# JuliaDSP/DSP.jl

Hardware: NVIDIA H100
Metric: Gsamples/s filt+welch on 2^26 cplx-F32 (higher is better)
Workload: dtype c64 (ComplexF32; f32 arithmetic)

## Files before the change

dsp.jl_b200/csrc/fft_core.cuh:

```cuda
#pragma once
#include "common.cuh"
#include <math.h>

#ifndef DSP_PROBE
#define DSP_PROBE 0
#endif

namespace dspb200 {

template <typename T> struct fft_pad { static constexpr int K = sizeof(T) == 4 ? 2 : 1; };
template <typename T> __host__ __device__ constexpr int fft_pad256(int n) {
    if (sizeof(T) == 4) return n == 512 ? 8 : (n == 1024 ? 4 : (n == 8192 ? 4 : 2));
    return n == 512 ? 4 : (n == 1024 ? 2 : (n == 8192 ? 2 : 1));
}
template <typename T> __host__ __device__ constexpr int fft_pad4096(int n) {
    if (sizeof(T) == 4) return n == 8192 ? 2 : (n == 16384 ? 4 : 0);
    return n == 8192 ? 1 : 0;
}
template <typename T, int N> __host__ __device__ __forceinline__ constexpr int padaddr(int p) {
    return p + fft_pad<T>::K * (p >> 4) + fft_pad256<T>(N) * (p >> 8) + fft_pad4096<T>(N) * (p >> 12);
}
template <typename T> __host__ __device__ constexpr int padded_len(int n) {
    return ((n - 1) + fft_pad<T>::K * ((n - 1) >> 4) + fft_pad256<T>(n) * ((n - 1) >> 8) + fft_pad4096<T>(n) * ((n - 1) >> 12) + 1 + 3) & ~3;
}
// ... 217 lines not shown
    if constexpr (fft_uses_t256<N>()) {
        for (int i = tid; i < fft_tw256_len(N); i += NT) s256[i] = g256[i];
    }
    if constexpr (fft_tl_in_smem<T, N>()) {
        cx<T>* sl = s256 + (fft_uses_t256<N>() ? fft_tw256_len(N) : 0);
        for (int i = tid; i < fft_tl_len<N>(); i += NT) sl[i] = gtl[i];
        c.tl = sl;
    }
    return c;
}
template <typename T, int N, int NT>
__device__ __forceinline__ FftCtx<T> fft_make_ctx(cx<T>* smem, const cx<T>* __restrict__ g16, const cx<T>* __restrict__ g256,
                                                    const cx<T>* __restrict__ gtl, int tid) {
    return fft_make_ctx_at<T, N, NT>(smem, smem + padded_len<T>(N), g16, g256, gtl, tid);
}

template <int NT> __device__ __forceinline__ void fft_group256_sync(int tid) {
#ifdef __CUDA_ARCH__
    if constexpr (NT <= 256) __syncthreads();
    else asm volatile("bar.sync %0, %1;" ::"r"(1 + (tid >> 8)), "r"(256) : "memory");
#endif
}

struct FftCtaScope {
    __device__ __forceinline__ void sync() const {
#ifdef __CUDA_ARCH__
        __syncthreads();
#endif
    }
};
template <int NTG> struct FftGroupScope {
    int id;
    __device__ __forceinline__ void sync() const {
#ifdef __CUDA_ARCH__
        asm volatile("bar.sync %0, %1;" ::"r"(id), "n"(NTG) : "memory");
#endif
    }
};

template <int NT> __device__ __forceinline__ void fft_gate_wait(int tid) {
#ifdef __CUDA_ARCH__
    if constexpr (NT > 256) {
        const int k = tid >> 8;
        if (k > 0) asm volatile("bar.sync %0, 512;" ::"r"(4 + k) : "memory");
    }
#endif
}
template <int NT> __device__ __forceinline__ void fft_gate_open(int tid) {
#ifdef __CUDA_ARCH__
    if constexpr (NT > 256) {
        const int k = tid >> 8;
        if (k < NT / 256 - 1) asm volatile("bar.arrive %0, 512;" ::"r"(5 + k) : "memory");
    }
#endif
}

template <typename T, int N> __host__ __device__ __forceinline__ void fft_store_block(cx<T>* sm, int cidx, const cx<T> (&v)[16]) {
    cx<T>* p = sm + padaddr<T, N>(16 * fft_block_of<N>(cidx));
#pragma unroll
    for (int r = 0; r < 16; r += 2) sts2<T>(p + r, v[r], v[r + 1]);
}

template <typename T, int N, int NT, bool SYNC, class Ld0, class Scope = FftCtaScope>
__host__ __device__ __forceinline__ void fft_first_pass(const FftCtx<T>& c, int tid, Ld0 ld0, Scope sc = Scope()) {
    constexpr int Q = fft_plan_traits<N>::Q;
    constexpr int ITERS = (Q + NT - 1) / NT;
#pragma unroll
    for (int it = 0; it < ITERS; ++it) {
        const int b = tid + it * NT;
        const bool active = (Q % NT == 0) || b < Q;
        cx<T> v[16];
        if (active) {
#pragma unroll
            for (int r = 0; r < 16; ++r) v[r] = ld0(b + r * Q, it, r);
            fft_bfly16_plain<T>(v);
        }
#ifdef __CUDA_ARCH__
        if constexpr (SYNC) { if (it == 0) sc.sync(); }
#endif
        if (active) fft_store_block<T, N>(c.sm, b, v);
    }
}

template <typename T, int N, int NT, bool SYNC, int ITERS, class Scope = FftCtaScope>
__device__ __forceinline__ void fft_first_pass_regs(const FftCtx<T>& c, int tid, cx<T> (&v)[ITERS][16], Scope sc = Scope()) {
    constexpr int Q = fft_plan_traits<N>::Q;
    static_assert(ITERS == (Q + NT - 1) / NT, "register tile does not match the thread count");
#pragma unroll
    for (int it = 0; it < ITERS; ++it) {
        const int b = tid + it * NT;
        const bool active = (Q % NT == 0) || b < Q;
        if (active) fft_bfly16_plain<T>(v[it]);
        if constexpr (SYNC) { if (it == 0) sc.sync(); }
        if (active) fft_store_block<T, N>(c.sm, b, v[it]);
    }
}

template <typename T, int N, int NT, int S, bool GATE = false>
__host__ __device__ __forceinline__ void fft_pass16(const FftCtx<T>& c, int tid) {
    static_assert(S == 16 || S == 256, "radix-16 pass with an unsupported stride");
    constexpr int Q = fft_plan_traits<N>::Q;
    constexpr int ITERS = (Q + NT - 1) / NT;
    constexpr int PS = padded_stride<T, N>(S);
    const cx<T>* tab = S == 16 ? c.t16 : c.t256;
    if constexpr (ITERS == 2 && Q % NT == 0) {
        const int b0 = tid, b1 = tid + NT;
        const int t0 = b0 & (S - 1), t1 = b1 & (S - 1);
        cx<T>* p0 = c.sm + padaddr<T, N>((b0 / S) * (16 * S) + t0);
        cx<T>* p1 = c.sm + padaddr<T, N>((b1 / S) * (16 * S) + t1);
        cx<T> v0[16], v1[16], w0[8], w1[8];
        if constexpr (GATE) fft_gate_wait<NT>(tid);
        load_tw8<T, S, fft_tw_row(N)>(tab, t0, w0);
#pragma unroll
        for (int r = 0; r < 16; ++r) v0[r] = p0[r * PS];
        load_tw8<T, S, fft_tw_row(N)>(tab, t1, w1);
#pragma unroll
        for (int r = 0; r < 16; ++r) v1[r] = p1[r * PS];
        if constexpr (GATE) fft_gate_open<NT>(tid);
        fft_bfly<T, 16, false>(v0, w0);
#pragma unroll
        for (int r = 0; r < 16; ++r) p0[r * PS] = v0[r];
        fft_bfly<T, 16, false>(v1, w1);
#pragma unroll
        for (int r = 0; r < 16; ++r) p1[r * PS] = v1[r];
        return;
    }
#pragma unroll 1
    for (int it = 0; it < ITERS; ++it) {
        const int b = tid + it * NT;
        if (Q % NT != 0 && b >= Q) break;
        const int t = b & (S - 1);
        cx<T>* p = c.sm + padaddr<T, N>((b / S) * (16 * S) + t);
        cx<T> v[16], w[8];
        if constexpr (GATE && ITERS == 1) fft_gate_wait<NT>(tid);
        load_tw8<T, S, fft_tw_row(N)>(tab, t, w);
#pragma unroll
        for (int r = 0; r < 16; ++r) v[r] = p[r * PS];
        if constexpr (GATE && ITERS == 1) fft_gate_open<NT>(tid);
        fft_bfly<T, 16, false>(v, w);
#pragma unroll
        for (int r = 0; r < 16; ++r) p[r * PS] = v[r];
    }
}

template <typename T, int N, int NT, class Scope = FftCtaScope>
__device__ __forceinline__ void fft_middle(const FftCtx<T>& c, int tid, Scope sc = Scope()) {
    constexpr int NMID = fft_plan_traits<N>::NMID;
    static_assert(NMID < 2 || std::is_same<Scope, FftCtaScope>::value, "thread groups run transforms of at most 4096 points");
    if constexpr (NMID >= 1) {
#if !(DSP_PROBE & 16)
        fft_pass16<T, N, NT, 16, true>(c, tid);
#endif
        if constexpr (NMID == 2) {
            fft_group256_sync<NT>(tid);
#if !(DSP_PROBE & 1)
            fft_pass16<T, N, NT, 256>(c, tid);
#endif
        }
        sc.sync();
    }
}

template <typename T, int N>
__host__ __device__ __forceinline__ void fft_last_pass_load(const FftCtx<T>& c, int tp, cx<T> (&v)[16]) {
    constexpr int Q = fft_plan_traits<N>::Q;
    const cx<T>* p = c.sm + padaddr<T, N>(tp);
#pragma unroll
    for (int r = 0; r < 16; ++r) v[r] = p[padaddr<T, N>(r * Q)];
}
template <typename T, int N>
__host__ __device__ __forceinline__ void fft_last_pass_bfly(const FftCtx<T>& c, int tp, cx<T> (&v)[16]) {
    using P = fft_plan_traits<N>;
    constexpr int Q = P::Q, RL = P::RL;
    if constexpr (RL == 16) {
        cx<T> w[8];
        load_tw8<T, Q, fft_tw_row(N)>(Q == 16 ? c.t16 : c.t256, tp, w);
        fft_bfly<T, 16, false>(v, w);
    } else {
        constexpr int NBF = 16 / RL;
        constexpr int TLK = P::TLK;
#pragma unroll
        for (int a = 0; a < NBF; ++a) {
            const int t = tp + Q * a;
            cx<T> w[RL / 2];
            if constexpr (N == 16384) {
                const cx<T> w1 = fft_tl_in_smem<T, N>() ? c.tl[t] : ldtw<T>(c.tl, t);
                w[1] = w1;
                w[0] = mkc<T>(fma_(w1.x, w1.x, -(w1.y * w1.y)), (w1.x + w1.x) * w1.y);
            } else {
#pragma unroll
                for (int i = 0; i < TLK; ++i) w[i] = fft_tl_in_smem<T, N>() ? c.tl[t * TLK + i] : ldtw<T>(c.tl, t * TLK + i);
            }
            cx<T> u[RL];
#pragma unroll
            for (int j = 0; j < RL; ++j) u[j] = v[a + NBF * j];
            fft_bfly<T, RL, false>(u, w);
#pragma unroll
            for (int j = 0; j < RL; ++j) v[a + NBF * j] = u[j];
        }
    }
}
template <typename T, int N, int GATE_NT = 0>
__host__ __device__ __forceinline__ void fft_last_pass(const FftCtx<T>& c, int tp, cx<T> (&v)[16], int tid = 0) {
    if constexpr (GATE_NT > 256) fft_gate_wait<GATE_NT>(tid);
    fft_last_pass_load<T, N>(c, tp, v);
    if constexpr (GATE_NT > 256) fft_gate_open<GATE_NT>(tid);
    fft_last_pass_bfly<T, N>(c, tp, v);
}

template <int N> struct fft_last_chunks {
    static constexpr int RL = fft_plan_traits<N>::RL;
    static constexpr int COUNT = 16 / RL;
};
template <typename T, int N, int A>
__device__ __forceinline__ void fft_last_pass_chunk(const FftCtx<T>& c, int tp, cx<T> (&u)[fft_plan_traits<N>::RL]) {
    using P = fft_plan_traits<N>;
    constexpr int Q = P::Q, RL = P::RL, NBF = 16 / RL;
    const cx<T>* p = c.sm + padaddr<T, N>(tp);
#pragma unroll
    for (int j = 0; j < RL; ++j) u[j] = p[padaddr<T, N>((A + NBF * j) * Q)];
    if constexpr (RL == 16) {
        cx<T> w[8];
        load_tw8<T, Q, fft_tw_row(N)>(Q == 16 ? c.t16 : c.t256, tp, w);
        fft_bfly<T, 16, false>(u, w);
    } else {
        const int t = tp + Q * A;
        cx<T> w[RL / 2];
        if constexpr (N == 16384) {
            const cx<T> w1 = fft_tl_in_smem<T, N>() ? c.tl[t] : ldtw<T>(c.tl, t);
            w[1] = w1;
            w[0] = mkc<T>(fma_(w1.x, w1.x, -(w1.y * w1.y)), (w1.x + w1.x) * w1.y);
        } else {
#pragma unroll
            for (int i = 0; i < P::TLK; ++i) w[i] = fft_tl_in_smem<T, N>() ? c.tl[t * P::TLK + i] : ldtw<T>(c.tl, t * P::TLK + i);
        }
        fft_bfly<T, RL, false>(u, w);
    }
}

template <typename T, int N, int NT, class Ld0, class StLast>
__device__ __forceinline__ void fft_forward(const FftCtx<T>& c, int tid, Ld0 ld0, StLast stlast) {
    constexpr int Q = fft_plan_traits<N>::Q;
    constexpr int ITERS = (Q + NT - 1) / NT;
    fft_first_pass<T, N, NT, false>(c, tid, ld0);
    __syncthreads();
    fft_middle<T, N, NT>(c, tid);
#pragma unroll
    for (int it = 0; it < ITERS; ++it) {
        const int tp = tid + it * NT;
        if (Q % NT != 0 && tp >= Q) break;
        cx<T> v[16];
        fft_last_pass<T, N>(c, tp, v);
#pragma unroll
        for (int r = 0; r < 16; ++r) stlast(tp + r * Q, it, r, v[r]);
    }
}

struct fft_r32 {
    static constexpr int N = 16384;
    static constexpr int NT = 512;
    static constexpr int Q = N / 32;
    static constexpr int QL = N / 16;
    static constexpr int T32_LEN = 32 * 16;
    static constexpr int TL_LEN = 2 * QL;
    static constexpr int TABLE_LEN = T32_LEN + TL_LEN;
    static constexpr int C10 = 2;
    static constexpr int PADDED_LEN = ((N - 1) + C10 * ((N - 1) >> 10) + 1 + 3) & ~3;
    static constexpr int SMEM_ELEMS = PADDED_LEN + TABLE_LEN;
};
__host__ __device__ __forceinline__ constexpr int fft_r32_padaddr(int p) { return p + fft_r32::C10 * (p >> 10); }
__host__ __device__ __forceinline__ constexpr int fft_r32_block_of(int c) { return 32 * (c & 15) + (c >> 4); }

template <typename T> struct FftR32Ctx {
    cx<T>* sm;
    const cx<T>* t32;
    const cx<T>* tl;
};
template <typename T>
__device__ __forceinline__ FftR32Ctx<T> fft_r32_make_ctx(cx<T>* data, cx<T>* tabs, const cx<T>* __restrict__ g, int tid) {
    for (int i = tid; i < fft_r32::TABLE_LEN; i += fft_r32::NT) tabs[i] = g[i];
    return FftR32Ctx<T>{data, tabs, tabs + fft_r32::T32_LEN};
}

// ... 125 lines not shown
```

dsp.jl_b200/csrc/spectral.cu:

```cuda
#include "fft_core.cuh"
#include "async_copy.cuh"
#include "cufft_exec.cuh"
#include <math.h>
#include <stdlib.h>
#include <new>
#include <vector>

namespace dspb200 {

struct SpecPlanImpl {
    int dtype = 0;
    bool cplx = false, f64 = false;
    int64_t n = 0, noverlap = 0, hop = 0, nfft = 0;
    int onesided = 0;
    int64_t nout = 0;
    bool fused = false;
    int device = 0;
    int sm_count = 0;
    void* d_window = nullptr;
    void* d_tw = nullptr;
    void* d_t32 = nullptr;
    void* d_t16 = nullptr;
    void* d_t256 = nullptr;
    size_t smem_optin = 0;
    int64_t ntapers = 0;
    DevBuf tmp;
    struct WelchCfg { void* kern = nullptr; size_t smem = 0; int g = 0, per_sm = 0, threads = 0, mode = -1; int64_t vctas = 0, used = 0; };
    WelchCfg welch_cfg[2];
    int nparts = 0;
    int rows_used = 0;
    DevBuf partial;
    WelchCfg welch_batch_cfg[2];
    WelchCfg welch_mt_cfg[2];
    DevBuf bpartial;
    DevBuf bacc;
    cufftHandle fft = 0;
    bool fft_ok = false;
    int64_t batch = 0;
    int64_t nbins_fft = 0;
    DevBuf segbuf, specbuf, acc;
    HostPipe pipe;
    DevBuf hin, hout;
    DevBuf seam;
    DevBuf y;
};

template <typename T> struct win_t { using type = double; };
template <> struct win_t<float> { using type = float2; };
__device__ __forceinline__ double win_mul(double v, double w) { return v * w; }
__device__ __forceinline__ float win_mul(float v, float2 w) { return fmaf(v, w.x, v * w.y); }

__device__ __forceinline__ float add_rn(float a, float b) { return __fadd_rn(a, b); }
__device__ __forceinline__ double add_rn(double a, double b) { return __dadd_rn(a, b); }

template <typename T, bool CPLX> struct in_type { using type = T; };
template <typename T> struct in_type<T, true> { using type = cx<T>; };

template <typename T, int N, bool CPLX, int MODE> struct welch_layout {
    using In = typename in_type<T, CPLX>::type;
    using W = typename win_t<T>::type;
    __host__ __device__ static size_t table_bytes() { return (size_t)fft_table_elems<T, N>() * sizeof(cx<T>); }
    __host__ __device__ static size_t window_bytes(int64_t n) { return MODE == 2 ? (size_t)n * sizeof(W) : 0; }
    __host__ __device__ static size_t stage_elems(int64_t n, int64_t hop) { return MODE >= 1 ? (size_t)(CPLX ? n : hop + n) : 0; }
    __host__ __device__ static size_t group_bytes(int64_t n, int64_t hop) {
        return (((size_t)padded_len<T>(N) * sizeof(cx<T>) + stage_elems(n, hop) * sizeof(In) + 15) & ~(size_t)15) + 16;
    }
    __host__ __device__ static size_t total(int64_t n, int64_t hop, int groups) {
        return table_bytes() + window_bytes(n) + (size_t)groups * group_bytes(n, hop);
    }
};
template <typename T, int N, int G> struct welch_bounds {
    static constexpr int NTG = fft_threads<N>::value;
    static constexpr int minblocks = G == 1 ? fft_minblocks<T, N>::value : 1;
};

struct Nil {};
template <bool USED, typename X> using welch_arg = typename std::conditional<USED, X, Nil>::type;

template <typename T, int N, bool CPLX, int MODE, int G, bool BATCH, bool TAPERS = false>
__global__ void __launch_bounds__((welch_bounds<T, N, G>::NTG * G), (welch_bounds<T, N, G>::minblocks))
welch_fused_kernel(const void* __restrict__ s_, welch_arg<BATCH, int64_t> chan_stride, welch_arg<!BATCH, int64_t> seg0,
                   int64_t nseg, welch_arg<BATCH, int64_t> upc, welch_arg<BATCH, int64_t> per, welch_arg<BATCH, int> slices,
                   welch_arg<BATCH, int64_t> nitems, int64_t hop, int n, welch_arg<!BATCH, int64_t> sample_offset,
                   const typename win_t<T>::type* __restrict__ win, const cx<T>* __restrict__ tw,
                   const cx<T>* __restrict__ g16, const cx<T>* __restrict__ g256, T* __restrict__ partial,
                   welch_arg<!BATCH, int> fresh_from) {
    constexpr int NT = fft_threads<N>::value;
    constexpr int NB16 = N / 16;
    constexpr int ITL = (NB16 + NT - 1) / NT;
    using L = welch_layout<T, N, CPLX, MODE>;
    using Scope = typename std::conditional<G == 1, FftCtaScope, FftGroupScope<NT>>::type;
    extern __shared__ __align__(16) unsigned char smem_raw[];
    using In = typename in_type<T, CPLX>::type;
    const In* s = reinterpret_cast<const In*>(s_);
    const int gid = G == 1 ? 0 : threadIdx.x / NT;
    const int tid = G == 1 ? threadIdx.x : threadIdx.x - gid * NT;
    constexpr bool TMA = MODE >= 1;
    constexpr bool WSM = MODE == 2;
    constexpr bool WREG = MODE == 3;
    static_assert(!TAPERS || (BATCH && MODE <= 1), "taper rows: the batched work assignment, window read per unit");
    using W = typename win_t<T>::type;
    cx<T>* tabs = reinterpret_cast<cx<T>*>(smem_raw);
    W* wsm = reinterpret_cast<W*>(smem_raw + L::table_bytes());
    unsigned char* gbase = smem_raw + L::table_bytes() + L::window_bytes(n) + (size_t)gid * L::group_bytes(n, hop);
    cx<T>* sm = reinterpret_cast<cx<T>*>(gbase);
    In* stage = reinterpret_cast<In*>(sm + padded_len<T>(N));
    uint64_t* bar = reinterpret_cast<uint64_t*>(gbase + L::group_bytes(n, hop) - 16);
    pdl_launch_dependents();
    const FftCtx<T> ctx = fft_make_ctx_at<T, N, NT * G>(sm, tabs, g16, g256, tw, threadIdx.x);
    if constexpr (WSM) {
        for (int i = threadIdx.x; i < n; i += NT * G) wsm[i] = win[i];
    }
    Scope scope;
    if constexpr (G > 1) scope.id = 8 + gid;
    W wreg[WREG ? ITL : 1][WREG ? 16 : 1];
    if constexpr (WREG) {
#pragma unroll
        for (int it = 0; it < ITL; ++it)
#pragma unroll
            for (int r = 0; r < 16; ++r) {
                const int j = tid + it * NT + r * NB16;
                wreg[it][r] = (j < n && tid + it * NT < NB16) ? win[j] : W{};
            }
    }

    T acc[ITL][16];
#pragma unroll
    for (int i = 0; i < ITL; ++i)
#pragma unroll
        for (int r = 0; r < 16; ++r) acc[i][r] = T(0);

    int64_t work;
    if constexpr (BATCH) work = nitems;
    else work = CPLX ? nseg : (nseg + 1) / 2;
    const int64_t vcta = (int64_t)blockIdx.x * G + gid, nvcta = (int64_t)gridDim.x * G;
    const int64_t share = (work + nvcta - 1) / nvcta;
    const int64_t w0 = vcta * share < work ? vcta * share : work;
    const int64_t w1 = w0 + share < work ? w0 + share : work;

    auto unit_src = [&](int64_t c, int64_t u) -> const In* {
        if constexpr (TAPERS) return s + c * chan_stride;
        else if constexpr (BATCH) return s + c * chan_stride + (CPLX ? u : 2 * u) * hop;
        else return s + ((seg0 + (CPLX ? u : 2 * u)) * hop - sample_offset);
    };
    auto unit_bytes = [&](int64_t u) -> uint32_t {
        const bool hasB = !CPLX && (2 * u + 1 < nseg);
        return (uint32_t)((hasB ? hop + n : n) * sizeof(In));
    };
    auto item_range = [&](int64_t i, int64_t& c, int64_t& ua, int64_t& ub) {
        if constexpr (BATCH) {
            c = i / slices;
            ua = (i - c * slices) * per;
            ub = ua + per < upc ? ua + per : upc;
        }
    };
    if constexpr (TMA) {
        if (tid == 0) {
            mbar_init(bar, 1);
            mbar_fence_init();
        }
    }
    pdl_wait();
    __syncthreads();
    int64_t c = 0, ua = BATCH ? 0 : w0, ub = BATCH ? 0 : w1;
    if constexpr (BATCH) {
        if (w0 < w1) item_range(w0, c, ua, ub);
    }
    if constexpr (TMA) {
        if (tid == 0 && w0 < w1) {
            mbar_expect_tx(bar, unit_bytes(ua));
            tma_load_1d(stage, unit_src(c, ua), unit_bytes(ua), bar);
        }
    }
    uint32_t parity = 0;

    for (int64_t item = w0; !BATCH || item < w1; ++item) {
        for (int64_t u = ua; u < ub; ++u) {
            const bool hasB = !CPLX && (2 * u + 1 < nseg);
            const In* pa = TMA ? stage : unit_src(c, u);
            const In* pb = pa + hop;
            const W* wu = TAPERS ? win + u * n : win;
            if constexpr (TMA) {
                if (!TAPERS || u == ua) {
                    mbar_wait(bar, parity);
                    parity ^= 1;
                }
            }
            auto ld0 = [&](int j, int it, int r) -> cx<T> {
                if (j >= n) return mkc<T>(T(0), T(0));
                if constexpr (CPLX) {
                    cx<T> v = pa[j];
                    if (WREG || WSM || wu) { const W w = WREG ? wreg[WREG ? it : 0][WREG ? r : 0] : (WSM ? wsm[j] : wu[j]); v = mkc<T>(win_mul(v.x, w), win_mul(v.y, w)); }
                    return v;
                } else {
                    T a = pa[j];
                    T b = hasB ? pb[j] : T(0);
                    if (WREG || WSM || wu) { const W w = WREG ? wreg[WREG ? it : 0][WREG ? r : 0] : (WSM ? wsm[j] : wu[j]); a = win_mul(a, w); b = win_mul(b, w); }
                    return mkc<T>(a, b);
                }
            };
            fft_first_pass<T, N, NT, true>(ctx, tid, ld0, scope);
            scope.sync();
            if constexpr (TMA && !BATCH) {
                if (tid == 0 && u + 1 < ub) {
                    fence_proxy_async_shared();
                    mbar_expect_tx(bar, unit_bytes(u + 1));
                    tma_load_1d(stage, unit_src(c, u + 1), unit_bytes(u + 1), bar);
                }
            }
            if constexpr (TMA && BATCH) {
                if (tid == 0) {
                    int64_t nc = c, nu = u + 1, nub = ub;
                    if (nu == ub && item + 1 < w1) item_range(item + 1, nc, nu, nub);
                    else if (TAPERS) nu = nub;
                    if (nu < nub) {
                        fence_proxy_async_shared();
                        mbar_expect_tx(bar, unit_bytes(nu));
                        tma_load_1d(stage, unit_src(nc, nu), unit_bytes(nu), bar);
                    }
                }
            }
            fft_middle<T, N, NT>(ctx, tid, scope);
#pragma unroll
            for (int it = 0; it < ITL; ++it) {
                const int tp = tid + it * NT;
                if (NB16 % NT != 0 && tp >= NB16) break;
                cx<T> v[16];
                fft_last_pass<T, N>(ctx, tp, v);
#pragma unroll
                for (int r = 0; r < 16; ++r) acc[it][r] += cabs2(v[r]);
            }
        }

        T* dst = partial + (BATCH ? item : vcta) * N;
        bool add = false;
        if constexpr (!BATCH) add = vcta < fresh_from;
#pragma unroll
        for (int it = 0; it < ITL; ++it) {
            const int tp = tid + it * NT;
            if (tp < NB16) {
#pragma unroll
                for (int r = 0; r < 16; ++r) {
                    if constexpr (BATCH) {
                        dst[tp + r * NB16] = acc[it][r];
                        acc[it][r] = T(0);
                    } else {
                        T* q = dst + tp + r * NB16;
                        *q = add ? *q + acc[it][r] : acc[it][r];
                    }
                }
            }
        }
        if constexpr (BATCH) {
            if (item + 1 < w1) item_range(item + 1, c, ua, ub);
        } else {
            break;
        }
    }
}

template <typename T, int N>
__global__ void __launch_bounds__(1024) welch_finalize_kernel(const T* __restrict__ partial, int rows, T* __restrict__ out,
                                                              int nout, int real_in, int onesided, double m1, double m2) {
    __shared__ double red[32][33];
    pdl_launch_dependents();
    pdl_wait();
    const int b = threadIdx.x & 31, sl = threadIdx.x >> 5, nw = blockDim.x >> 5;
    const int k = blockIdx.x * 32 + b;
    const T* chan = partial + (int64_t)blockIdx.y * rows * N;
    double sum = 0.0;
    if (k < nout) {
        const T* c0 = chan + k;
        const T* c1 = chan + ((N - k) & (N - 1));
        if (real_in) {
            for (int c = sl; c < rows; c += nw) sum += (double)c0[(int64_t)c * N] + (double)c1[(int64_t)c * N];
        } else {
            for (int c = sl; c < rows; c += nw) sum += (double)c0[(int64_t)c * N];
        }
    }
    red[sl][b] = sum;
    __syncthreads();
    if (sl == 0 && k < nout) {
        for (int i = 1; i < nw; ++i) sum += red[i][b];
        double m = m1;
        if (real_in) {
            sum *= 0.5;
// ... 631 lines not shown
        }
        red[which][sl][b] = sum;
    };
    part(rows, ri, 0);
    part(seam_rows, rs, 1);
    __syncthreads();
    if (sl == 0 && k < nout) {
        const int nwi = ri < 32 ? ri : 32, nws = rs < 32 ? rs : 32;
        double sum = red[0][0][b];
        for (int i = 1; i < nwi; ++i) sum += red[0][i][b];
        if (rs > 0) {
            double s2 = red[1][0][b];
            for (int i = 1; i < nws; ++i) s2 += red[1][i][b];
            sum += s2;
        }
        double* q = acc + (int64_t)blockIdx.y * nout + k;
        *q = add ? *q + sum : sum;
    }
}

template <typename T>
__global__ void welch_stream_acc_kernel(const cx<T>* __restrict__ X, int64_t nbins_fft, int64_t nfft, int64_t nout, int64_t f0,
                                        int64_t nf, int64_t k, int add, double* __restrict__ acc) {
    const int64_t kk = (int64_t)blockIdx.x * blockDim.x + threadIdx.x;
    if (kk >= nout) return;
    const int64_t c = f0 / k + blockIdx.y;
    const int64_t a = c * k > f0 ? c * k : f0, e = (c + 1) * k < f0 + nf ? (c + 1) * k : f0 + nf;
    const int64_t src = kk < nbins_fft ? kk : nfft - kk;
    double sum = 0.0;
    for (int64_t f = a; f < e; ++f) sum += (double)cabs2(X[(f - f0) * nbins_fft + src]);
    double* q = acc + c * nout + kk;
    *q = (add || a > c * k) ? *q + sum : sum;
}

template <typename T>
__global__ void welch_stream_power_kernel(const double* __restrict__ acc, int64_t nout, int64_t nfft, int onesided, int half,
                                          double m1, double m2, T* __restrict__ out) {
    const int64_t kk = (int64_t)blockIdx.x * blockDim.x + threadIdx.x;
    if (kk >= nout) return;
    const int64_t i = (int64_t)blockIdx.y * nout + kk;
    double sum = acc[i];
    if (half) sum *= 0.5;
    const double m = (onesided && kk != 0 && 2 * kk != nfft) ? m2 : m1;
    out[i] = (T)(sum * m);
}

static bool fused_size_ok(int64_t nfft, bool f64) {
    if (nfft < 256 || (nfft & (nfft - 1))) return false;
    return nfft <= (f64 ? 8192 : 16384);
}

template <typename T, typename F> static int fused_size_dispatch(const SpecPlanImpl* p, const char* what, F&& f) {
    switch (p->nfft) {
#define X(NN)                                                                                               \
    case NN:                                                                                                \
        if constexpr (sizeof(T) == 8 && NN > 8192) break;                                                   \
        else return f(T(0), std::integral_constant<int, NN>());
        X(256) X(512) X(1024) X(2048) X(4096) X(8192) X(16384)
#undef X
    }
    set_error("no fused %s kernel for nfft=%lld", what, (long long)p->nfft);
    return DSPB200_EUNSUPPORTED;
}
template <typename F> static int fused_dispatch(const SpecPlanImpl* p, const char* what, F&& f) {
    return p->f64 ? fused_size_dispatch<double>(p, what, f) : fused_size_dispatch<float>(p, what, f);
}

template <typename K> static int set_smem(K kernel, size_t bytes) {
    if (bytes > 48 * 1024) DSP_CUDA(cudaFuncSetAttribute(kernel, cudaFuncAttributeMaxDynamicSharedMemorySize, (int)bytes));
    return DSPB200_OK;
}

template <typename T, bool BATCH>
using welch_kern_t = void (*)(const void*, welch_arg<BATCH, int64_t>, welch_arg<!BATCH, int64_t>, int64_t,
                              welch_arg<BATCH, int64_t>, welch_arg<BATCH, int64_t>, welch_arg<BATCH, int>,
                              welch_arg<BATCH, int64_t>, int64_t, int, welch_arg<!BATCH, int64_t>,
                              const typename win_t<T>::type*, const cx<T>*, const cx<T>*, const cx<T>*, T*,
                              welch_arg<!BATCH, int>);

template <typename T, int N, bool CPLX, bool BATCH, bool TAPERS, typename F>
static int welch_candidates(const SpecPlanImpl* p, bool aligned, bool windowed, F&& f) {
    constexpr bool MULTI = sizeof(T) == 4 && N >= 1024 && N <= 4096;
    constexpr bool WREGOK = sizeof(T) == 4 && N <= 4096;
#define DSP_WELCH_CAND(MODE_, G_)                                                                                   \
    DSP_TRY(f(welch_kern_t<T, BATCH>(welch_fused_kernel<T, N, CPLX, MODE_, G_, BATCH, TAPERS>),                     \
              welch_layout<T, N, CPLX, MODE_>::total(p->n, p->hop, G_), MODE_, G_))
    if (aligned) {
        if constexpr (!TAPERS) {
            if (windowed) {
                if constexpr (CPLX) {
                    if constexpr (WREGOK) DSP_WELCH_CAND(3, 1);
                    DSP_WELCH_CAND(2, 1);
                    if constexpr (MULTI) { DSP_WELCH_CAND(3, 2); DSP_WELCH_CAND(2, 2); }
                } else {
                    if constexpr (MULTI) { DSP_WELCH_CAND(2, 3); DSP_WELCH_CAND(2, 2); }
                    DSP_WELCH_CAND(2, 1);
                    if constexpr (WREGOK) DSP_WELCH_CAND(3, 1);
                }
            }
        }
        if constexpr (MULTI && !CPLX) DSP_WELCH_CAND(1, 3);
        DSP_WELCH_CAND(1, 1);
        if constexpr (MULTI) DSP_WELCH_CAND(1, 2);
    }
    DSP_WELCH_CAND(0, 1);
#undef DSP_WELCH_CAND
    return DSPB200_OK;
}

template <typename K>
static int welch_per_sm(const SpecPlanImpl* p, K k, int threads, int g, size_t smem, int64_t row_cap, int* per_sm) {
    DSP_TRY(set_smem(k, smem));
    DSP_CUDA(cudaOccupancyMaxActiveBlocksPerMultiprocessor(per_sm, k, threads, smem));
    if (row_cap > 0 && (int64_t)*per_sm * g * p->sm_count > row_cap) *per_sm = (int)(row_cap / ((int64_t)g * p->sm_count));
    return DSPB200_OK;
}

template <typename T, int N, bool CPLX, bool BATCH, bool TAPERS = false>
static int welch_select(SpecPlanImpl* p, SpecPlanImpl::WelchCfg& cfg, bool aligned, int64_t row_cap) {
    if (cfg.kern != nullptr) return DSPB200_OK;
    constexpr int NT = fft_threads<N>::value;
    using Kern = welch_kern_t<T, BATCH>;
    struct Cand { Kern k; size_t smem; int mode, g, warps, per_sm; };
    Cand best{nullptr, 0, 0, 0, -1, 0};
    auto consider = [&](Kern k, size_t smem, int mode, int g) -> int {
        if (best.warps >= 12 || (mode == 0 && best.k != nullptr)) return DSPB200_OK;
        if (smem > p->smem_optin) return DSPB200_OK;
        int per_sm = 0;
        DSP_TRY(welch_per_sm(p, k, NT * g, g, smem, row_cap, &per_sm));
        if (per_sm < 1) return DSPB200_OK;
        const int warps = per_sm * g * NT / 32;
        if (warps > best.warps) best = Cand{k, smem, mode, g, warps, per_sm};
        return DSPB200_OK;
    };
    DSP_TRY((welch_candidates<T, N, CPLX, BATCH, TAPERS>(p, aligned, p->d_window != nullptr, consider)));
    DSP_REQUIRE(best.k != nullptr, "no %sWelch kernel configuration fits (nfft=%lld)", BATCH ? "batched " : "", (long long)p->nfft);
    DSP_TRY(set_smem(best.k, best.smem));
    cfg.kern = reinterpret_cast<void*>(best.k); cfg.smem = best.smem; cfg.g = best.g; cfg.per_sm = best.per_sm;
    cfg.threads = NT * best.g; cfg.mode = best.mode;
    return DSPB200_OK;
}

static int64_t welch_wave(const SpecPlanImpl* p, const SpecPlanImpl::WelchCfg& cfg) {
    return cfg.vctas ? cfg.vctas / cfg.g : (int64_t)p->sm_count * cfg.per_sm;
}

template <typename T, bool BATCH>
static int welch_launch(SpecPlanImpl* p, SpecPlanImpl::WelchCfg& cfg, int64_t work, const void* s,
                        welch_arg<BATCH, int64_t> chan_stride, welch_arg<!BATCH, int64_t> seg0, int64_t nseg,
                        welch_arg<BATCH, int64_t> upc, welch_arg<BATCH, int64_t> per, welch_arg<BATCH, int> slices,
                        welch_arg<BATCH, int64_t> nitems, welch_arg<!BATCH, int64_t> sample_offset, void* partial,
                        welch_arg<!BATCH, int> fresh_from, cudaStream_t st) {
    const int64_t wave = welch_wave(p, cfg), want = cdiv(work, cfg.g);
    const int grid = (int)(want < wave ? want : wave);
    DSP_CUDA(launch_pdl(reinterpret_cast<welch_kern_t<T, BATCH>>(cfg.kern), (unsigned)grid, (unsigned)cfg.threads, cfg.smem, st,
                        s, chan_stride, seg0, nseg, upc, per, slices, nitems, p->hop, (int)p->n, sample_offset,
                        reinterpret_cast<const typename win_t<T>::type*>(p->d_window), reinterpret_cast<const cx<T>*>(p->d_tw),
                        reinterpret_cast<const cx<T>*>(p->d_t16), reinterpret_cast<const cx<T>*>(p->d_t256),
                        reinterpret_cast<T*>(partial), fresh_from));
    DSP_LAUNCH_OK();
    cfg.used = (int64_t)grid * cfg.g;
    return DSPB200_OK;
}

template <typename T, int N, bool CPLX>
static int launch_welch_fused(SpecPlanImpl* p, const void* s, int64_t seg0, int64_t nseg, int64_t sample_offset,
                              cudaStream_t st) {
    using In = typename in_type<T, CPLX>::type;
    const uintptr_t first = (uintptr_t)s + (uintptr_t)((seg0 * p->hop - sample_offset) * (int64_t)sizeof(In));
    const bool aligned = (first % 16 == 0) && ((p->hop * sizeof(In)) % 16 == 0) && ((p->n * sizeof(In)) % 16 == 0);
    const int64_t units = CPLX ? nseg : (nseg + 1) / 2;
    if (units < 1) return DSPB200_OK;
    SpecPlanImpl::WelchCfg& cfg = p->welch_cfg[aligned ? 1 : 0];
    DSP_TRY((welch_select<T, N, CPLX, false>(p, cfg, aligned, p->nparts)));
    DSP_TRY((welch_launch<T, false>(p, cfg, cfg.vctas ? cfg.vctas : units, s, Nil(), seg0, nseg, Nil(), Nil(), Nil(), Nil(),
                                    sample_offset, p->partial.p, p->rows_used, st)));
    if (cfg.used > p->rows_used) p->rows_used = (int)cfg.used;
    return DSPB200_OK;
}

template <typename T, int N>
static int launch_welch_finalize(SpecPlanImpl* p, double r, void* out, cudaStream_t st) {
    DSP_CUDA(launch_pdl(welch_finalize_kernel<T, N>, (unsigned)cdiv(p->nout, 32), 1024u, (size_t)0, st,
                        reinterpret_cast<const T*>(p->partial.p), p->rows_used, reinterpret_cast<T*>(out), (int)p->nout,
                        p->cplx ? 0 : 1, (int)p->onesided, 1.0 / r, 2.0 / r));
    DSP_LAUNCH_OK();
    return DSPB200_OK;
}

static constexpr size_t WELCH_BATCH_SCRATCH = (size_t)32 << 20;

static int64_t welch_batch_slices(int64_t gc, int64_t upc, int64_t nv, int64_t max_slices) {
    int64_t lim = upc < max_slices ? upc : max_slices;
    if (lim > 2 * nv) lim = 2 * nv;
    int64_t best = 1, best_cost = cdiv(gc, nv) * upc;
    for (int64_t sl = 2; sl <= lim; ++sl) {
        const int64_t per = cdiv(upc, sl);
        if (cdiv(upc, per) != sl) continue;
        const int64_t cost = cdiv(gc * sl, nv) * per;
        if (cost < best_cost) { best = sl; best_cost = cost; }
    }
    return best;
}

static bool welch_batch_aligned(const SpecPlanImpl* p, const void* s, int64_t stride, int64_t nchan, size_t esz) {
    return ((uintptr_t)s % 16 == 0) && ((stride * (int64_t)esz) % 16 == 0 || nchan == 1) && ((p->hop * (int64_t)esz) % 16 == 0) &&
           ((p->n * (int64_t)esz) % 16 == 0);
}

struct WelchBatchWork { int64_t k = 0, upc = 0, slices = 0, per = 0, nitems = 0; };
static WelchBatchWork welch_batch_work(const SpecPlanImpl* p, const SpecPlanImpl::WelchCfg& cfg, bool cplx, int64_t gc, int64_t k,
                                       int64_t max_slices) {
    WelchBatchWork w;
    w.k = k;
// ... 42 lines not shown

template <typename T, int N, bool CPLX>
static int launch_stft_fused(SpecPlanImpl* p, const void* s, int64_t len, int64_t nchan, int64_t k, double r,
                             int psd_only, void* out, cudaStream_t st, const StftStreamArgs& sa) {
    constexpr int NT = fft_threads<N>::value;
    using In = typename in_type<T, CPLX>::type;
    using SS = StftStream<In>;
    const size_t base = (size_t)fft_smem_elems<T, N>() * sizeof(cx<T>);
    const size_t stage = (size_t)(CPLX ? p->n : p->hop + p->n) * sizeof(In) + 16;
    constexpr bool W1K = sizeof(T) == 4 && N == 1024;
    const bool plan_aligned = ((p->hop * sizeof(In)) % 16 == 0) && ((p->n * sizeof(In)) % 16 == 0);
    const bool aligned = plan_aligned && ((uintptr_t)s % 16 == 0) && ((len * sizeof(In)) % 16 == 0 || nchan == 1) &&
                         (sa.h * sizeof(In)) % 16 == 0;
    const bool tma = !W1K && aligned &&
                     (base + stage <= p->smem_optin) && (base + stage <= 100 * 1024 || N >= 8192);
    const size_t smem = tma ? base + stage : base;
    const int64_t upc = CPLX ? k : (k + 1) / 2;
    const int64_t units = upc * nchan;
    if (units < 1) return DSPB200_OK;
    const SS ss{reinterpret_cast<const In*>(sa.seam), sa.lds, sa.h, sa.ldo, (W1K ? aligned : tma) ? 1 : 0, sa.ntapers};
    const auto* w = reinterpret_cast<const typename win_t<T>::type*>(p->d_window);
    const bool mt = sa.ntapers > 0;
    if constexpr (W1K) {
        if ((sa.keep_plan ? plan_aligned : aligned) && p->d_t32 != nullptr) {
            constexpr int WARPS = 4;
            const size_t smem1 = (size_t)w1k::T32_LEN * sizeof(cx<float>) + (w && !mt ? (size_t)p->n * sizeof(float2) : 0) +
                                 (size_t)WARPS * w1k::warp_bytes(CPLX ? p->n : p->hop + p->n, sizeof(In));
            using K1 = void (*)(const void*, int64_t, int64_t, int64_t, int64_t, int64_t, int, const float2*, const cx<float>*, void*, int,
                                int, int, float, float, SS);
            K1 k1 = mt ? (K1)stft_w1k_kernel<CPLX, 2, WARPS> : w ? (K1)stft_w1k_kernel<CPLX, 1, WARPS> : (K1)stft_w1k_kernel<CPLX, 0, WARPS>;
            if (smem1 <= p->smem_optin) {
                DSP_TRY(set_smem(k1, smem1));
                int per = 1;
                DSP_CUDA(cudaOccupancyMaxActiveBlocksPerMultiprocessor(&per, k1, 32 * WARPS, smem1));
                const int64_t cap1 = (int64_t)p->sm_count * (per < 1 ? 1 : per);
                const int64_t want = cdiv(units, WARPS);
                const unsigned grid1 = (unsigned)(want < cap1 ? want : cap1);
                k1<<<grid1, 32 * WARPS, smem1, st>>>(s, len, k, upc, units, p->hop, (int)p->n, reinterpret_cast<const float2*>(w),
                                                      reinterpret_cast<const cx<float>*>(p->d_t32), out, (int)p->nout, psd_only,
                                                      p->onesided, (float)(1.0 / r), (float)(2.0 / r), ss);
                DSP_LAUNCH_OK();
                return DSPB200_OK;
            }
        }
    }
    const auto* tw = reinterpret_cast<const cx<T>*>(p->d_tw);
    const auto* g16 = reinterpret_cast<const cx<T>*>(p->d_t16);
    const auto* g256 = reinterpret_cast<const cx<T>*>(p->d_t256);
    using Kern = void (*)(const void*, int64_t, int64_t, int64_t, int64_t, int64_t, int, const typename win_t<T>::type*, const cx<T>*,
                          const cx<T>*, const cx<T>*, void*, int, int, int, T, T, SS);
    constexpr bool SPEC = sizeof(T) == 4;
    Kern kern;
    if (mt) {
        if constexpr (W1K) kern = (Kern)stft_fused_kernel<T, N, CPLX, false, 2>;
        else kern = tma ? (Kern)stft_fused_kernel<T, N, CPLX, true, 2> : (Kern)stft_fused_kernel<T, N, CPLX, false, 2>;
    } else if constexpr (W1K) {
        kern = w ? (Kern)stft_fused_kernel<T, N, CPLX, false, 1> : (Kern)stft_fused_kernel<T, N, CPLX, false, 0>;
    } else if constexpr (SPEC) {
        if (tma) kern = w ? (Kern)stft_fused_kernel<T, N, CPLX, true, 1> : (Kern)stft_fused_kernel<T, N, CPLX, true, 0>;
        else kern = w ? (Kern)stft_fused_kernel<T, N, CPLX, false, 1> : (Kern)stft_fused_kernel<T, N, CPLX, false, 0>;
    } else {
        kern = tma ? (Kern)stft_fused_kernel<T, N, CPLX, true, -1> : (Kern)stft_fused_kernel<T, N, CPLX, false, -1>;
    }
    DSP_TRY(set_smem(kern, smem));
    int per_sm = 1;
    DSP_CUDA(cudaOccupancyMaxActiveBlocksPerMultiprocessor(&per_sm, kern, NT, smem));
    const int64_t cap = (int64_t)p->sm_count * (per_sm < 1 ? 1 : per_sm);
    const unsigned grid = (unsigned)(units < cap ? units : cap);
    kern<<<grid, NT, smem, st>>>(s, len, k, upc, units, p->hop, (int)p->n, w, tw, g16, g256, out, (int)p->nout, psd_only,
                                 p->onesided, (T)(1.0 / r), (T)(2.0 / r), ss);
    DSP_LAUNCH_OK();
    return DSPB200_OK;
}

template <typename T, int N, bool CPLX, bool BATCH, bool TAPERS = false>
static int welch_pin(SpecPlanImpl* p, int mode, int g, int64_t vctas) {
    constexpr int NT = fft_threads<N>::value;
    using Kern = welch_kern_t<T, BATCH>;
    SpecPlanImpl::WelchCfg pinned[2];
    for (int a = 0; a < 2; ++a) {
        const int m = a ? mode : 0, gg = a ? g : 1;
        Kern k = nullptr;
        size_t smem = 0;
        DSP_TRY((welch_candidates<T, N, CPLX, BATCH, TAPERS>(p, true, true, [&](Kern kc, size_t sc, int mc, int gc) -> int {
            if (mc == m && gc == gg) { k = kc; smem = sc; }
            return DSPB200_OK;
        })));
        if (k == nullptr) {
            set_error("no Welch kernel instance MODE %d, G %d for this plan (nfft=%lld)", m, gg, (long long)N);
            return DSPB200_EUNSUPPORTED;
        }
        if (m >= 2 && p->d_window == nullptr) {
            set_error("Welch MODE %d needs a window", m);
            return DSPB200_EUNSUPPORTED;
        }
        if (smem > p->smem_optin) {
            set_error("Welch MODE %d, G %d needs %zu bytes of shared memory (limit %zu)", m, gg, smem, p->smem_optin);
            return DSPB200_EUNSUPPORTED;
        }
        int per_sm = 0;
        DSP_TRY(welch_per_sm(p, k, NT * gg, gg, smem, !BATCH && vctas == 0 ? p->nparts : 0, &per_sm));
        if (per_sm < 1) {
            set_error("Welch MODE %d, G %d does not fit an SM", m, gg);
            return DSPB200_EUNSUPPORTED;
        }
        pinned[a].kern = reinterpret_cast<void*>(k); pinned[a].smem = smem; pinned[a].g = gg; pinned[a].per_sm = per_sm;
        pinned[a].threads = NT * gg; pinned[a].mode = m; pinned[a].vctas = vctas;
    }
    SpecPlanImpl::WelchCfg* cfg = TAPERS ? p->welch_mt_cfg : BATCH ? p->welch_batch_cfg : p->welch_cfg;
    cfg[0] = pinned[0];
    cfg[1] = pinned[1];
    return DSPB200_OK;
}

static int generic_prepare(SpecPlanImpl* p) {
    if (p->fft_ok) return DSPB200_OK;
    int64_t b = (int64_t(1) << 22) / p->nfft;
    if (b < 1) b = 1;
    if (b > 8192) b = 8192;
    p->batch = b;
    DSP_TRY(fft_plan_1d(&p->fft, p->cplx, p->f64, CUFFT_FORWARD, p->nfft, b));
    p->fft_ok = true;
    const size_t esz = dtype_size(p->dtype);
    DSP_TRY(p->segbuf.reserve((size_t)(b * p->nfft) * esz));
    DSP_TRY(p->specbuf.reserve((size_t)(b * p->nbins_fft) * (p->f64 ? 16 : 8)));
    DSP_TRY(p->acc.reserve((size_t)p->nbins_fft * sizeof(double)));
    return DSPB200_OK;
}

template <typename T> static int generic_segments(SpecPlanImpl* p, const void* s, int64_t first_sample, int64_t nseg,
                                                   cudaStream_t st) {
    const int64_t total = p->batch * p->nfft;
    const int threads = 256;
    const int grid = (int)(cdiv(total, threads) < 65535 * 8 ? cdiv(total, threads) : 65535 * 8);
    if (p->cplx)
        seg_window_kernel<T, true><<<grid, threads, 0, st>>>(s, first_sample, p->hop, p->n, p->nfft, nseg, p->batch, reinterpret_cast<const typename win_t<T>::type*>(p->d_window), p->segbuf.p);
    else
        seg_window_kernel<T, false><<<grid, threads, 0, st>>>(s, first_sample, p->hop, p->n, p->nfft, nseg, p->batch, reinterpret_cast<const typename win_t<T>::type*>(p->d_window), p->segbuf.p);
    DSP_LAUNCH_OK();
    return fft_exec(p->fft, p->cplx, p->f64, CUFFT_FORWARD, p->segbuf.p, p->specbuf.p, st);
}

template <typename T> static int welch_generic_acc(SpecPlanImpl* p, const void* s, int64_t sample_offset,
                                                    int64_t seg_begin, int64_t seg_end, cudaStream_t st) {
    for (int64_t b0 = seg_begin; b0 < seg_end; b0 += p->batch) {
        const int64_t nseg = seg_end - b0 < p->batch ? seg_end - b0 : p->batch;
        DSP_TRY(generic_segments<T>(p, s, b0 * p->hop - sample_offset, nseg, st));
        const int threads = 128;
        pow_acc_kernel<T><<<(int)cdiv(p->nbins_fft, threads), threads, 0, st>>>(
            reinterpret_cast<const cx<T>*>(p->specbuf.p), p->nbins_fft, nseg, reinterpret_cast<double*>(p->acc.p));
        DSP_LAUNCH_OK();
    }
    return DSPB200_OK;
}

static unsigned stream_generic_cols(const SpecPlanImpl* p, int64_t len, int threads) {
    const int64_t want = cdiv(len, threads), cap = cdiv((int64_t)p->sm_count * 16, p->batch);
    return (unsigned)(want < cap ? want : cap);
}

template <typename T> static int stream_generic_fft(SpecPlanImpl* p, const void* hist, int64_t h, int64_t ldh, const void* x,
                                                     int64_t nx, int64_t f0, int64_t nf, int64_t k, cudaStream_t st) {
    const int threads = 256;
    const auto* w = reinterpret_cast<const typename win_t<T>::type*>(p->d_window);
    const dim3 gseg(stream_generic_cols(p, p->nfft, threads), (unsigned)p->batch);
    if (p->cplx)
        stft_seg_kernel<T, true><<<gseg, threads, 0, st>>>(hist, h, ldh, x, nx, f0, nf, k, p->hop, p->n, p->nfft, w, p->segbuf.p);
// ... 1067 lines not shown
```

Before: 76.47.

## Process overlapping Welch segment pairs per CTA with shared staging and twiddles

Adds a MODE 4 Welch kernel for complex F32 4096-point FFTs with 50% overlap. Each iteration stages two overlapping segments (hop+n samples) with one TMA load and runs both transforms in double-sized shared memory. The pair shares twiddle loads and windowed input registers. This is meant to cut global reads and per-segment sync overhead, at the cost of more shared memory, one block per SM in launch bounds, and higher register pressure.

```diff
diff --git a/dsp.jl_b200/csrc/fft_core.cuh b/dsp.jl_b200/csrc/fft_core.cuh
--- a/dsp.jl_b200/csrc/fft_core.cuh
+++ b/dsp.jl_b200/csrc/fft_core.cuh
@@ -323,10 +323,19 @@
     }
 }
 
-template <typename T, int N, int NT, bool SYNC, int ITERS, class Scope = FftCtaScope>
+template <typename T, int N, int NT, bool SYNC, int ITERS, class Scope = FftCtaScope, int PAIR = 0>
 __device__ __forceinline__ void fft_first_pass_regs(const FftCtx<T>& c, int tid, cx<T> (&v)[ITERS][16], Scope sc = Scope()) {
     constexpr int Q = fft_plan_traits<N>::Q;
-    static_assert(ITERS == (Q + NT - 1) / NT, "register tile does not match the thread count");
+    if constexpr (PAIR > 0) {
+        static_assert(ITERS == 2 && Q == NT, "a pair of transforms: one butterfly of each per thread");
+        fft_bfly16_plain<T>(v[0]);
+        fft_bfly16_plain<T>(v[1]);
+        if constexpr (SYNC) sc.sync();
+        fft_store_block<T, N>(c.sm, tid, v[0]);
+        fft_store_block<T, N>(c.sm + PAIR, tid, v[1]);
+        return;
+    }
+    static_assert(PAIR > 0 || ITERS == (Q + NT - 1) / NT, "register tile does not match the thread count");
 #pragma unroll
     for (int it = 0; it < ITERS; ++it) {
         const int b = tid + it * NT;
@@ -337,31 +346,32 @@
     }
 }
 
-template <typename T, int N, int NT, int S, bool GATE = false>
+template <typename T, int N, int NT, int S, bool GATE = false, int PAIR = 0>
 __host__ __device__ __forceinline__ void fft_pass16(const FftCtx<T>& c, int tid) {
     static_assert(S == 16 || S == 256, "radix-16 pass with an unsupported stride");
     constexpr int Q = fft_plan_traits<N>::Q;
     constexpr int ITERS = (Q + NT - 1) / NT;
     constexpr int PS = padded_stride<T, N>(S);
     const cx<T>* tab = S == 16 ? c.t16 : c.t256;
-    if constexpr (ITERS == 2 && Q % NT == 0) {
-        const int b0 = tid, b1 = tid + NT;
+    if constexpr (PAIR > 0 || (ITERS == 2 && Q % NT == 0)) {
+        static_assert(PAIR == 0 || Q == NT, "a pair of transforms: one butterfly of each per thread");
+        const int b0 = tid, b1 = PAIR > 0 ? tid : tid + NT;
         const int t0 = b0 & (S - 1), t1 = b1 & (S - 1);
         cx<T>* p0 = c.sm + padaddr<T, N>((b0 / S) * (16 * S) + t0);
-        cx<T>* p1 = c.sm + padaddr<T, N>((b1 / S) * (16 * S) + t1);
+        cx<T>* p1 = c.sm + PAIR + padaddr<T, N>((b1 / S) * (16 * S) + t1);
         cx<T> v0[16], v1[16], w0[8], w1[8];
         if constexpr (GATE) fft_gate_wait<NT>(tid);
         load_tw8<T, S, fft_tw_row(N)>(tab, t0, w0);
 #pragma unroll
         for (int r = 0; r < 16; ++r) v0[r] = p0[r * PS];
-        load_tw8<T, S, fft_tw_row(N)>(tab, t1, w1);
+        if constexpr (PAIR == 0) load_tw8<T, S, fft_tw_row(N)>(tab, t1, w1);
 #pragma unroll
         for (int r = 0; r < 16; ++r) v1[r] = p1[r * PS];
         if constexpr (GATE) fft_gate_open<NT>(tid);
         fft_bfly<T, 16, false>(v0, w0);
 #pragma unroll
         for (int r = 0; r < 16; ++r) p0[r * PS] = v0[r];
-        fft_bfly<T, 16, false>(v1, w1);
+        fft_bfly<T, 16, false>(v1, PAIR > 0 ? w0 : w1);
 #pragma unroll
         for (int r = 0; r < 16; ++r) p1[r * PS] = v1[r];
         return;
@@ -384,18 +394,18 @@
     }
 }
 
-template <typename T, int N, int NT, class Scope = FftCtaScope>
+template <typename T, int N, int NT, class Scope = FftCtaScope, int PAIR = 0>
 __device__ __forceinline__ void fft_middle(const FftCtx<T>& c, int tid, Scope sc = Scope()) {
     constexpr int NMID = fft_plan_traits<N>::NMID;
     static_assert(NMID < 2 || std::is_same<Scope, FftCtaScope>::value, "thread groups run transforms of at most 4096 points");
     if constexpr (NMID >= 1) {
 #if !(DSP_PROBE & 16)
-        fft_pass16<T, N, NT, 16, true>(c, tid);
+        fft_pass16<T, N, NT, 16, true, PAIR>(c, tid);
 #endif
         if constexpr (NMID == 2) {
             fft_group256_sync<NT>(tid);
 #if !(DSP_PROBE & 1)
-            fft_pass16<T, N, NT, 256>(c, tid);
+            fft_pass16<T, N, NT, 256, false, PAIR>(c, tid);
 #endif
         }
         sc.sync();
@@ -440,6 +450,19 @@
             for (int j = 0; j < RL; ++j) v[a + NBF * j] = u[j];
         }
     }
+}
+template <typename T, int N, int PAIR>
+__device__ __forceinline__ void fft_last_pass_pair(const FftCtx<T>& c, int tp, cx<T> (&va)[16], cx<T> (&vb)[16]) {
+    using P = fft_plan_traits<N>;
+    static_assert(P::RL == 16, "a pair of transforms whose last pass is a radix-16 pass");
+    FftCtx<T> cb = c;
+    cb.sm += PAIR;
+    fft_last_pass_load<T, N>(c, tp, va);
+    fft_last_pass_load<T, N>(cb, tp, vb);
+    cx<T> w[8];
+    load_tw8<T, P::Q, fft_tw_row(N)>(P::Q == 16 ? c.t16 : c.t256, tp, w);
+    fft_bfly<T, 16, false>(va, w);
+    fft_bfly<T, 16, false>(vb, w);
 }
 template <typename T, int N, int GATE_NT = 0>
 __host__ __device__ __forceinline__ void fft_last_pass(const FftCtx<T>& c, int tp, cx<T> (&v)[16], int tid = 0) {
diff --git a/dsp.jl_b200/csrc/spectral.cu b/dsp.jl_b200/csrc/spectral.cu
--- a/dsp.jl_b200/csrc/spectral.cu
+++ b/dsp.jl_b200/csrc/spectral.cu
@@ -59,11 +59,14 @@
 template <typename T, int N, bool CPLX, int MODE> struct welch_layout {
     using In = typename in_type<T, CPLX>::type;
     using W = typename win_t<T>::type;
+    static constexpr int NBUF = MODE == 4 ? 2 : 1;
     __host__ __device__ static size_t table_bytes() { return (size_t)fft_table_elems<T, N>() * sizeof(cx<T>); }
     __host__ __device__ static size_t window_bytes(int64_t n) { return MODE == 2 ? (size_t)n * sizeof(W) : 0; }
-    __host__ __device__ static size_t stage_elems(int64_t n, int64_t hop) { return MODE >= 1 ? (size_t)(CPLX ? n : hop + n) : 0; }
+    __host__ __device__ static size_t stage_elems(int64_t n, int64_t hop) {
+        return MODE >= 1 ? (size_t)(CPLX && MODE != 4 ? n : hop + n) : 0;
+    }
     __host__ __device__ static size_t group_bytes(int64_t n, int64_t hop) {
-        return (((size_t)padded_len<T>(N) * sizeof(cx<T>) + stage_elems(n, hop) * sizeof(In) + 15) & ~(size_t)15) + 16;
+        return (((size_t)NBUF * padded_len<T>(N) * sizeof(cx<T>) + stage_elems(n, hop) * sizeof(In) + 15) & ~(size_t)15) + 16;
     }
     __host__ __device__ static size_t total(int64_t n, int64_t hop, int groups) {
         return table_bytes() + window_bytes(n) + (size_t)groups * group_bytes(n, hop);
@@ -78,7 +81,7 @@
 template <bool USED, typename X> using welch_arg = typename std::conditional<USED, X, Nil>::type;
 
 template <typename T, int N, bool CPLX, int MODE, int G, bool BATCH, bool TAPERS = false>
-__global__ void __launch_bounds__((welch_bounds<T, N, G>::NTG * G), (welch_bounds<T, N, G>::minblocks))
+__global__ void __launch_bounds__((welch_bounds<T, N, G>::NTG * G), (MODE == 4 ? 1 : welch_bounds<T, N, G>::minblocks))
 welch_fused_kernel(const void* __restrict__ s_, welch_arg<BATCH, int64_t> chan_stride, welch_arg<!BATCH, int64_t> seg0,
                    int64_t nseg, welch_arg<BATCH, int64_t> upc, welch_arg<BATCH, int64_t> per, welch_arg<BATCH, int> slices,
                    welch_arg<BATCH, int64_t> nitems, int64_t hop, int n, welch_arg<!BATCH, int64_t> sample_offset,
@@ -97,14 +100,17 @@
     const int tid = G == 1 ? threadIdx.x : threadIdx.x - gid * NT;
     constexpr bool TMA = MODE >= 1;
     constexpr bool WSM = MODE == 2;
-    constexpr bool WREG = MODE == 3;
+    constexpr bool WREG = MODE >= 3;
+    constexpr bool PAIR = MODE == 4;
+    constexpr int PL = padded_len<T>(N);
     static_assert(!TAPERS || (BATCH && MODE <= 1), "taper rows: the batched work assignment, window read per unit");
+    static_assert(!PAIR || (sizeof(T) == 4 && CPLX && N == 4096 && G == 1 && !BATCH), "pairs: complex Float32 4096-point, one signal");
     using W = typename win_t<T>::type;
     cx<T>* tabs = reinterpret_cast<cx<T>*>(smem_raw);
     W* wsm = reinterpret_cast<W*>(smem_raw + L::table_bytes());
     unsigned char* gbase = smem_raw + L::table_bytes() + L::window_bytes(n) + (size_t)gid * L::group_bytes(n, hop);
     cx<T>* sm = reinterpret_cast<cx<T>*>(gbase);
-    In* stage = reinterpret_cast<In*>(sm + padded_len<T>(N));
+    In* stage = reinterpret_cast<In*>(sm + L::NBUF * padded_len<T>(N));
     uint64_t* bar = reinterpret_cast<uint64_t*>(gbase + L::group_bytes(n, hop) - 16);
     pdl_launch_dependents();
     const FftCtx<T> ctx = fft_make_ctx_at<T, N, NT * G>(sm, tabs, g16, g256, tw, threadIdx.x);
@@ -166,16 +172,23 @@
     if constexpr (BATCH) {
         if (w0 < w1) item_range(w0, c, ua, ub);
     }
+    auto span_bytes = [&](int64_t u) -> uint32_t { return (uint32_t)((u + 1 < ub ? hop + n : n) * sizeof(In)); };
     if constexpr (TMA) {
         if (tid == 0 && w0 < w1) {
-            mbar_expect_tx(bar, unit_bytes(ua));
-            tma_load_1d(stage, unit_src(c, ua), unit_bytes(ua), bar);
+            if constexpr (PAIR) {
+                mbar_expect_tx(bar, span_bytes(ua));
+                tma_load_1d(stage, unit_src(c, ua), span_bytes(ua), bar);
+            } else {
+                mbar_expect_tx(bar, unit_bytes(ua));
+                tma_load_1d(stage, unit_src(c, ua), unit_bytes(ua), bar);
+            }
         }
     }
     uint32_t parity = 0;
 
     for (int64_t item = w0; !BATCH || item < w1; ++item) {
-        for (int64_t u = ua; u < ub; ++u) {
+        for (int64_t u = ua; u < ub; u += PAIR ? 2 : 1) {
+            const bool two = PAIR && u + 1 < ub;
             const bool hasB = !CPLX && (2 * u + 1 < nseg);
             const In* pa = TMA ? stage : unit_src(c, u);
             const In* pb = pa + hop;
@@ -199,9 +212,43 @@
                     return mkc<T>(a, b);
                 }
             };
-            fft_first_pass<T, N, NT, true>(ctx, tid, ld0, scope);
-            scope.sync();
-            if constexpr (TMA && !BATCH) {
+            if constexpr (PAIR) {
+                if (two) {
+                    cx<T> x[24], v[2][16];
+#pragma unroll
+                    for (int m = 0; m < 24; ++m) x[m] = pa[tid + m * NB16];
+#pragma unroll
+                    for (int r = 0; r < 16; ++r) {
+                        const W w = wreg[0][r];
+                        v[0][r] = mkc<T>(win_mul(x[r].x, w), win_mul(x[r].y, w));
+                        v[1][r] = mkc<T>(win_mul(x[r + 8].x, w), win_mul(x[r + 8].y, w));
+                    }
+                    fft_first_pass_regs<T, N, NT, true, 2, Scope, PL>(ctx, tid, v, scope);
+                } else {
+                    fft_first_pass<T, N, NT, true>(ctx, tid, ld0, scope);
+                }
+                scope.sync();
+                const int64_t next = u + (two ? 2 : 1);
+                if (tid == 0 && next < ub) {
+                    fence_proxy_async_shared();
+                    mbar_expect_tx(bar, span_bytes(next));
+                    tma_load_1d(stage, unit_src(c, next), span_bytes(next), bar);
+                }
+                if (two) {
+                    fft_middle<T, N, NT, Scope, PL>(ctx, tid, scope);
+                    cx<T> va[16], vb[16];
+                    fft_last_pass_pair<T, N, PL>(ctx, tid, va, vb);
+#pragma unroll
+                    for (int r = 0; r < 16; ++r) acc[0][r] += cabs2(va[r]);
+#pragma unroll
+                    for (int r = 0; r < 16; ++r) acc[0][r] += cabs2(vb[r]);
+                    continue;
+                }
+            } else {
+                fft_first_pass<T, N, NT, true>(ctx, tid, ld0, scope);
+                scope.sync();
+            }
+            if constexpr (TMA && !BATCH && !PAIR) {
                 if (tid == 0 && u + 1 < ub) {
                     fence_proxy_async_shared();
                     mbar_expect_tx(bar, unit_bytes(u + 1));
@@ -999,14 +1046,21 @@
 static int welch_candidates(const SpecPlanImpl* p, bool aligned, bool windowed, F&& f) {
     constexpr bool MULTI = sizeof(T) == 4 && N >= 1024 && N <= 4096;
     constexpr bool WREGOK = sizeof(T) == 4 && N <= 4096;
-#define DSP_WELCH_CAND(MODE_, G_)                                                                                   \
-    DSP_TRY(f(welch_kern_t<T, BATCH>(welch_fused_kernel<T, N, CPLX, MODE_, G_, BATCH, TAPERS>),                     \
-              welch_layout<T, N, CPLX, MODE_>::total(p->n, p->hop, G_), MODE_, G_))
+    constexpr bool PAIROK = sizeof(T) == 4 && N == 4096 && CPLX && !BATCH && !TAPERS;
+#define DSP_WELCH_CAND_AS(KMODE_, MODE_, G_, SEGS_)                                                                 \
+    DSP_TRY(f(welch_kern_t<T, BATCH>(welch_fused_kernel<T, N, CPLX, KMODE_, G_, BATCH, TAPERS>),                    \
+              welch_layout<T, N, CPLX, KMODE_>::total(p->n, p->hop, G_), MODE_, G_, SEGS_))
+#define DSP_WELCH_CAND(MODE_, G_) DSP_WELCH_CAND_AS(MODE_, MODE_, G_, 1)
     if (aligned) {
         if constexpr (!TAPERS) {
             if (windowed) {
                 if constexpr (CPLX) {
-                    if constexpr (WREGOK) DSP_WELCH_CAND(3, 1);
+                    if constexpr (PAIROK) {
+                        if (p->n == N && 2 * p->hop == N) DSP_WELCH_CAND_AS(4, 3, 1, 2);
+                        else DSP_WELCH_CAND(3, 1);
+                    } else if constexpr (WREGOK) {
+                        DSP_WELCH_CAND(3, 1);
+                    }
                     DSP_WELCH_CAND(2, 1);
                     if constexpr (MULTI) { DSP_WELCH_CAND(3, 2); DSP_WELCH_CAND(2, 2); }
                 } else {
@@ -1022,6 +1076,7 @@
     }
     DSP_WELCH_CAND(0, 1);
 #undef DSP_WELCH_CAND
+#undef DSP_WELCH_CAND_AS
     return DSPB200_OK;
 }
 
@@ -1040,13 +1095,13 @@
     using Kern = welch_kern_t<T, BATCH>;
     struct Cand { Kern k; size_t smem; int mode, g, warps, per_sm; };
     Cand best{nullptr, 0, 0, 0, -1, 0};
-    auto consider = [&](Kern k, size_t smem, int mode, int g) -> int {
+    auto consider = [&](Kern k, size_t smem, int mode, int g, int segs) -> int {
         if (best.warps >= 12 || (mode == 0 && best.k != nullptr)) return DSPB200_OK;
         if (smem > p->smem_optin) return DSPB200_OK;
         int per_sm = 0;
         DSP_TRY(welch_per_sm(p, k, NT * g, g, smem, row_cap, &per_sm));
         if (per_sm < 1) return DSPB200_OK;
-        const int warps = per_sm * g * NT / 32;
+        const int warps = per_sm * g * segs * NT / 32;
         if (warps > best.warps) best = Cand{k, smem, mode, g, warps, per_sm};
         return DSPB200_OK;
     };
@@ -1255,7 +1310,7 @@
         const int m = a ? mode : 0, gg = a ? g : 1;
         Kern k = nullptr;
         size_t smem = 0;
-        DSP_TRY((welch_candidates<T, N, CPLX, BATCH, TAPERS>(p, true, true, [&](Kern kc, size_t sc, int mc, int gc) -> int {
+        DSP_TRY((welch_candidates<T, N, CPLX, BATCH, TAPERS>(p, true, true, [&](Kern kc, size_t sc, int mc, int gc, int) -> int {
             if (mc == m && gc == gg) { k = kc; smem = sc; }
             return DSPB200_OK;
         })));
```

New measurement: 77.81 (median of 6 runs). +1.8%, better.
